# thangvubk/SoftGroup

Measured on AMD Instinct MI355X. Metric: scans/sec ScanNet-v2-like inference (softgroup_scannet.yaml, full forward_test), higher is better.
Workload: dtype f32

## Files before the change

include/softgroup_hip.h:

```cpp
#ifndef SOFTGROUP_HIP_H
#define SOFTGROUP_HIP_H

#include <stddef.h>
#include <stdint.h>

#ifdef __cplusplus
extern "C" {
#endif

typedef void *sg_stream_t;

#define SG_OK 0
#define SG_ERR_ARG (-1)
#define SG_ERR_WORKSPACE (-2)
#define SG_ERR_LAUNCH (-3)
#define SG_ERR_UNSUPPORTED (-4)

#define SG_BALLQUERY_MAX_NEIGHBORS 1000
#define SG_OCTREE_NUM_NODES 585
#define SG_OCTREE_NUM_LEAVES 512
#define SG_LISTS_SORTED 1
#define SG_LISTS_RADIUS 2

int sg_version(void);
// ... 192 lines not shown
  const float *w2;
  const float *w_i;
} sg_unet_block;
typedef struct sg_unet_level {
  int planes, n_blocks;
  const sg_unet_block *blocks;
  const sg_unet_block *tail;
  const float *down_bn_scale, *down_bn_shift, *down_w;
  const float *up_bn_scale, *up_bn_shift, *up_w;
} sg_unet_level;
typedef struct sg_unet_desc {
  int n_levels;
  const sg_unet_level *levels;
  int input_cin;
  const float *input_w;
  const float *out_bn_scale, *out_bn_shift;
  int input_cin_packed;
  int arithmetic;
} sg_unet_desc;
size_t sg_unet_arena_bytes(const sg_unet_desc *desc, int num_rows);
int sg_unet_forward(const sg_unet_desc *desc, const float *feats, const int32_t *indices,
                    int num_rows, const int32_t *spatial_shape_host, float *out, void *arena,
                    size_t arena_bytes, sg_stream_t stream);

typedef struct sg_train_bn {
  const float *weight, *bias;
  float *running_mean, *running_var;
  float momentum, eps;
  float *g_weight, *g_bias;
} sg_train_bn;
typedef struct sg_train_conv {
  const float *w;
  float *g_w;
} sg_train_conv;
typedef struct sg_unet_train_block {
  int cin, cout;
  sg_train_bn bn1, bn2;
  sg_train_conv c1, c2, ci;
} sg_unet_train_block;
typedef struct sg_unet_train_level {
  int planes, n_blocks;
  const sg_unet_train_block *blocks, *tail;
  sg_train_bn down_bn, up_bn;
  sg_train_conv down, up;
} sg_unet_train_level;
typedef struct sg_unet_train_desc {
// ... 418 lines not shown
```

softgroup_amd/_lib.py:

```python
import ctypes as C
import os

_HERE = os.path.dirname(os.path.abspath(__file__))
LIB_PATH = os.path.join(_HERE, 'lib', os.environ.get('SG_LIB_NAME', 'libsoftgroup_hip.so'))

_lib = None

_vp, _i, _f, _i64, _sz, _d = C.c_void_p, C.c_int, C.c_float, C.c_int64, C.c_size_t, C.c_double
_pi32 = C.POINTER(C.c_int32)

SIGNATURES = {
    'sg_version': (_i, []),
    'sg_last_error': (C.c_char_p, []),
    'sg_device_info': (_i, [C.c_char_p, _i, C.POINTER(_i), C.POINTER(_i)]),
    'sg_stream_release': (_i, [_vp]),
    'sg_host_copy_2d': (_i, [_vp, _i64, _vp, _i64, _i64, _i64]),
    'sg_host_cast_f64_f32': (_i, [_vp, _vp, _i64]),
    'sg_host_fill_i64_strided': (_i, [_vp, _i64, _i64, _i64]),
    'sg_host_colmax_i64': (_i, [_vp, _i64, _i64, _vp]),
    'sg_stream_create': (_i, [_vp]),
    'sg_stream_create_priority': (_i, [_vp, _i]),
    'sg_stream_destroy': (_i, [_vp]),
    'sg_voxelize_idx_host': (_i, [_vp, _i, _i, _i, _vp, _pi32, _pi32]),
    'sg_voxelize_idx_fill_host': (_i, [_vp, _i, _i, _i, _vp, _i, _i, _vp, _vp]),
# ... 27 lines not shown
    'sg_get_mask_iou_on_pred': (_i, [_vp, _vp, _vp, _vp, _vp, _i, _i, _vp, _vp]),
    'sg_get_mask_label': (_i, [_vp, _vp, _vp, _vp, _vp, _i, _i, _f, _vp, _vp]),
    'sg_spconv_hash_workspace_bytes': (_sz, [_i]),
    'sg_spconv_subm_rulebook': (_i, [_vp, _i, _pi32, _vp, _vp, _sz, _vp]),
    'sg_spconv_pyramid_workspace_bytes': (_sz, [_i, _i]),
    'sg_spconv_pyramid_rows': (_i, [_vp, _i, _pi32, _i, _vp, _vp, _sz, _vp]),
    'sg_spconv_pyramid_build_workspace_bytes': (_sz, [_vp, _i]),
    'sg_spconv_pyramid_build': (_i, [_vp, _i, _pi32, _i, _vp, _vp, _sz, _vp, _sz, _vp]),
    'sg_spconv_down_build': (_i, [_vp, _i, _pi32, _vp, _vp, _vp, _sz, _vp]),
    'sg_spconv_down_fill': (_i, [_vp, _i, _vp, _i, _vp, _vp, _vp, _sz, _vp]),
    'sg_spconv_inverse_rulebook': (_i, [_vp, _vp, _i, _vp, _vp]),
    'sg_spconv_plan_workspace_bytes': (_sz, [_i]),
    'sg_spconv_plan': (_i, [_vp, _i, _i, _vp, _vp, _vp, _vp, _sz, _vp]),
    'sg_spconv_set_arithmetic': (_i, [_i]),
    'sg_spconv_set_combine': (_i, [_i]),
    'sg_spconv_set_chain': (_i, [_i]),
    'sg_grouping_set_lanes': (_i, [_i]),
    'sg_spconv_chain_stats': (_i, [_vp, _vp]),
    'sg_spconv_profile': (_i, [_i]),
    'sg_spconv_profile_read': (_i, [_vp, _vp]),
    'sg_spconv_profile_detail': (_i, [_vp, _vp, _i, _vp]),
    'sg_unet_arena_bytes': (_sz, [_vp, _i]),
    'sg_unet_forward': (_i, [_vp, _vp, _vp, _i, _vp, _vp, _vp, _sz, _vp]),
    'sg_unet_train_arena_hint': (_sz, [_vp, _i]),
    'sg_unet_train_forward': (_i, [_vp, _vp, _vp, _i, _vp, _vp, _vp, _sz, _vp, _vp, _vp]),
    'sg_unet_train_backward': (_i, [_vp, _vp, _vp, _vp]),
    'sg_unet_train_release': (None, [_vp]),
    'sg_pointwise_heads': (_i, [_vp, _vp, _i, _i, _i, _vp, _vp, _vp, _vp, _vp, _vp, _vp]),
    'sg_spconv_packed_weight_elems': (_sz, [_i, _i, _i]),
    'sg_spconv_pack_weight': (_i, [_vp, _i, _i, _i, _i, _vp, _vp]),
    'sg_spconv_conv_workspace_bytes': (_sz, [_i, _i]),
    'sg_spconv_gather_conv_f32': (_i, [_vp, _i, _vp, _i, _i, _i, _i, _vp, _vp, _vp, _vp, _vp, _vp,
                                       _vp, _vp, _vp, _vp, _vp, _vp, _sz, _vp]),
    'sg_spconv_packed_weight_elems_bf16': (_sz, [_i, _i, _i]),
    'sg_spconv_pack_weight_bf16': (_i, [_vp, _i, _i, _i, _i, _vp, _vp]),
    'sg_spconv_conv_bf16_workspace_bytes': (_sz, [_i, _i]),
    'sg_spconv_gather_conv_bf16': (_i, [_vp, _i, _vp, _i, _i, _i, _i, _vp, _vp, _vp, _vp, _vp, _vp, _sz,
                                        _vp]),
    'sg_spconv_transpose_table': (_i, [_vp, _i, _i, _vp, _vp]),
    'sg_spconv_wgrad_workspace_bytes': (_sz, [_i, _i, _i, _i]),
    'sg_spconv_wgrad': (_i, [_vp, _i, _vp, _i, _vp, _i, _i, _i, _i, _vp, _vp, _sz, _vp]),
    'sg_instance_npoint': (_i, [_vp, _vp, _i64, _i, _i, _f, _i, _vp, _vp]),
    'sg_instance_runs_workspace_bytes': (_sz, [_i, _i]),
    'sg_instance_runs': (_i, [_vp, _vp, _i64, _i, _i, _f, _vp, _i, _i, _i, _vp, _vp, _vp, _i64, _vp, _sz, _vp]),
    'sg_rle_format_bound': (_i64, [_i64, _i]),
    'sg_rle_format_host': (_i, [_vp, _vp, _vp, _i, _vp, _i64, _vp]),
# ... 150 lines not shown
```

softgroup_amd/build.py:

```python
import os
import subprocess
import sys
from concurrent.futures import ThreadPoolExecutor

HERE = os.path.dirname(os.path.abspath(__file__))
CSRC = os.path.join(HERE, 'csrc')
LIBDIR = os.path.join(HERE, 'lib')
OBJDIR = os.path.join(LIBDIR, 'obj')
LIB = os.path.join(LIBDIR, 'libsoftgroup_hip.so')
HIPCC = os.environ.get('HIPCC', '/opt/rocm/bin/hipcc')

SOURCES = [
    ('core.hip', ['-ffp-contract=off']),
    ('seg_ops.hip', ['-ffp-contract=off']),
    ('voxelize_idx.hip', ['-ffp-contract=off']),
    ('ballquery.hip', ['-ffp-contract=off']),
    ('octree.hip', ['-ffp-contract=off']),
    ('bfs.hip', ['-ffp-contract=off']),
    ('spconv_rulebook.hip', ['-ffp-contract=off']),
    ('spconv_conv.hip', ['-mllvm', '-amdgpu-mfma-vgpr-form', '-mllvm', '-amdgpu-atomic-optimizer-strategy=None'] + os.environ.get('SG_CONV_EXTRA_FLAGS', '').split()),
    ('spconv_train.hip', ['-mllvm', '-amdgpu-mfma-vgpr-form']),
    ('unet_exec.hip', ['-ffp-contract=off']),
    ('unet_train.hip', ['-ffp-contract=off']),
    ('instances.hip', ['-ffp-contract=off']),
    ('scan_exec.hip', ['-ffp-contract=off']),
    ('scan_forward.hip', ['-ffp-contract=off']),
    ('heads.hip', ['-ffp-contract=off']),
    ('eval_ops.hip', ['-ffp-contract=off']),
    ('inst_eval.hip', ['-ffp-contract=off']),
    ('det_eval.hip', ['-ffp-contract=off']),
    ('train_data.hip', ['-ffp-contract=off']),
    ('result_io.hip', ['-ffp-contract=off']),
    ('viz_io.hip', ['-ffp-contract=off']),
    ('mask_nms.hip', ['-ffp-contract=off']),
    ('resample.hip', ['-ffp-contract=off']),
    ('losses.hip', ['-ffp-contract=off']),
    ('optim.hip', ['-ffp-contract=off']),
    ('host_ops.cpp', ['-ffp-contract=off']),
]
COMMON = ['-O3', '-std=c++17', '-fPIC', '--offload-arch=gfx950', '-Wall', '-Wno-unused-function',
          '-Wno-unused-result', '-Wno-unused-value']


def _deps_mtime():
    m = 0
# ... 46 lines not shown
```

softgroup_amd/csrc/common.h:

```cpp
#pragma once
#include <hip/hip_runtime.h>
#include <stdint.h>
#include <stdio.h>

#include "../../include/softgroup_hip.h"

namespace sg {

constexpr int kWave = 64;

void set_error(const char *fmt, ...);
int32_t *pinned_words();

inline hipStream_t as_stream(sg_stream_t s) { return reinterpret_cast<hipStream_t>(s); }

inline int check_launch(const char *what) {
  hipError_t e = hipGetLastError();
  if (e != hipSuccess) {
    set_error("%s: %s", what, hipGetErrorString(e));
    return SG_ERR_LAUNCH;
  }
  return SG_OK;
}

// ... 142 lines not shown
  size_t mx = 0;
  for (int i = 0; i < f.n; ++i) mx = f.words[i] > mx ? f.words[i] : mx;
  const int gx = grid_for(static_cast<int64_t>(mx / 4 + 1), 256, 1024);
  fill_many_kernel<<<dim3(gx, f.n), 256, 0, stream>>>(f);
}

extern thread_local int t_conv_arith;
void conv_chain_begin(hipStream_t stream);
bool conv_chain_recording();
int conv_chain_end();
void conv_chain_abort();
int conv_chain_concat(const float *a, const float *b, int64_t rows, int ca, int cb, const float *scale,
                      const float *shift, float *out, float *out_act);
int conv_chain_bn_relu(const float *x, const float *scale, const float *shift, int64_t rows, int c, float *out);
int conv_chain_check_abort(const char *who);
int conv_gather_rows(const void *in, int num_in_rows, const int32_t *nbr, int M_out, int K, int Cin, int Cout,
                     const float *w_k8, const float *post_scale, const float *post_shift, const void *residual,
                     const float *act_scale, const float *act_shift, void *out_act, const int32_t *order,
                     const uint32_t *tile_mask, const int32_t *nbr_tiles, void *out, void *ws, size_t ws_bytes,
                     sg_stream_t stream, int in16, int out16, int res16);
int spconv_wgrad_layout(const void *in, int in_bf16, const void *g_out, int g_bf16, const int32_t *nbr_t, int M_out,
                        int K, int Cin, int Cout, float *dw, int out_oki, void *ws, size_t ws_bytes,
                        sg_stream_t stream);
struct PackJob {
  const float *w;
  float *out;
  int cout, kvol, cin, mode;
};
int spconv_pack_weights(const PackJob *jobs, int n, sg_stream_t stream);
size_t octree_stash_bytes(int n);
int octree_ballquery_count_stash(const float *points, const float *boxes, const int32_t *pt_inds,
                                 const int32_t *pt_start_len, int n, float radius, int32_t *start_len, int32_t *stash,
                                 hipStream_t stream);
int octree_ballquery_fill_stash(const float *points, const float *boxes, const int32_t *pt_inds,
                                const int32_t *pt_start_len, int n, float radius, const int32_t *start_len,
                                const int32_t *stash, int32_t *idx, hipStream_t stream);
void conv_release_stream(int dev, hipStream_t stream);
void unet_release_stream(int dev, hipStream_t stream);
void scan_release_stream(int dev, hipStream_t stream);
void bfs_release_stream(int dev, hipStream_t stream);
constexpr int kBfsGiantMin = 16384;
struct BfsDefer {
  bool deferred = false;
  hipStream_t side = nullptr;
};
void bfs_emit_defer(BfsDefer *d);
// ... 7 lines not shown
```

softgroup_amd/csrc/spconv_conv.hip:

```cpp
#include <stdlib.h>

#include <atomic>
#include <cstdio>
#include <map>
#include <mutex>
#include <utility>
#include <vector>

#include "common.h"

namespace sg {

typedef float f32x16 __attribute__((ext_vector_type(16)));
typedef float f4 __attribute__((ext_vector_type(4)));
typedef float f2 __attribute__((ext_vector_type(2)));
typedef __bf16 bf16x8 __attribute__((ext_vector_type(8)));
typedef __bf16 bf16x2 __attribute__((ext_vector_type(2)));

__device__ __forceinline__ void split3(const float (&x)[8], bf16x8 &h, bf16x8 &m, bf16x8 &l) {
#pragma unroll
  for (int j = 0; j < 4; ++j) {
    const f2 v = {x[2 * j], x[2 * j + 1]};
    const bf16x2 hh = __builtin_convertvector(v, bf16x2);
    const f2 r = v - __builtin_convertvector(hh, f2);
    const bf16x2 mm = __builtin_convertvector(r, bf16x2);
    const f2 r2 = r - __builtin_convertvector(mm, f2);
    const bf16x2 ll = __builtin_convertvector(r2, bf16x2);
    h[2 * j] = hh[0]; h[2 * j + 1] = hh[1];
    m[2 * j] = mm[0]; m[2 * j + 1] = mm[1];
    l[2 * j] = ll[0]; l[2 * j + 1] = ll[1];
  }
}
__device__ __forceinline__ bf16x8 round_bf16(const float (&x)[8]) {
  bf16x8 h;
#pragma unroll
  for (int j = 0; j < 4; ++j) {
    const f2 v = {x[2 * j], x[2 * j + 1]};
    const bf16x2 hh = __builtin_convertvector(v, bf16x2);
    h[2 * j] = hh[0]; h[2 * j + 1] = hh[1];
  }
  return h;
}
__device__ __forceinline__ uint16_t bf16_rne(float x) {
  const uint32_t u = __builtin_bit_cast(uint32_t, x);
  return static_cast<uint16_t>((u + 0x7fffu + ((u >> 16) & 1u)) >> 16);
}
__device__ __forceinline__ float bf16_f32(uint16_t b) {
  return __builtin_bit_cast(float, static_cast<uint32_t>(b) << 16);
}

#ifndef SG_WHATIF
#define SG_WHATIF 0
#endif

constexpr int kTileRows = 32;
// ... 1402 lines not shown
#define SG_B16_DEPTH 2
#endif
#ifndef SG_B16_WPE_PLUS
#define SG_B16_WPE_PLUS 0
#endif
template <int CK, int WPE, int NBW, int WV, int AT>
constexpr PersistentFn r16_variant() {
  if constexpr (AT) return gather_conv_persistent_kernel<CK, SG_B16_DEPTH, 0, WPE + SG_B16_WPE_PLUS, NBW, 2, WV, 1, 1>;
  else return nullptr;
}
#define SG_SPLIT_VARIANT(CK, DEPTH, WPE, NBW, WV, AT)                                            \
  {gather_conv_persistent_kernel<CK, DEPTH, 0, WPE, NBW, 1, WV, AT>,                              \
   gather_conv_persistent_kernel<CK, DEPTH, 1, WPE, NBW, 1, WV, AT>,                              \
   gather_conv_persistent_kernel<CK, SG_B16_DEPTH, 0, WPE + SG_B16_WPE_PLUS, NBW, 2, WV, AT>,     \
   r16_variant<CK, WPE, NBW, WV, AT>(), NBW, WV, CK, AT, 0, 0, 0, 0}
constexpr int kSplitVariants = 9;
static SplitVariant g_split_variants[kSplitVariants] = {
    SG_SPLIT_VARIANT(32, 2, 2, 2, 2, 1),  SG_SPLIT_VARIANT(32, 2, 3, 1, 2, 1),
    SG_SPLIT_VARIANT(32, 2, 2, 2, 4, 1),  SG_SPLIT_VARIANT(32, 2, 3, 1, 4, 1), SG_SPLIT_VARIANT(32, 2, 1, 1, 8, 1),
    SG_SPLIT_VARIANT(16, 2, 3, 2, 4, 0),  SG_SPLIT_VARIANT(16, 2, 4, 1, 4, 0), SG_SPLIT_VARIANT(16, 2, 2, 1, 8, 0),
    SG_SPLIT_VARIANT(16, 2, 1, 1, 16, 0),
};

static int launch_persistent_split(ConvArgs a, int num_tiles, long long in_bytes, long long w_bytes,
                                   hipStream_t stream, bool b16, bool in16) {
  static int num_cu = 0;
  static std::once_flag once;
  std::call_once(once, [] {
    int dev = 0;
    hipGetDevice(&dev);
    hipDeviceGetAttribute(&num_cu, hipDeviceAttributeMultiprocessorCount, dev);
    if (num_cu <= 0) num_cu = 256;
    auto prepare = [](SplitVariant &v) {
      v.lds = static_cast<size_t>(v.wv) * v.nbw * 16 * 64 * sizeof(float) + 2 * kMetaInts * sizeof(int32_t) + 16 +
              (v.at ? static_cast<size_t>(v.wv) * 4096 : 0);
      int o = 0;
      hipOccupancyMaxActiveBlocksPerMultiprocessor(&o, v.fn, 64 * v.wv, v.lds);
      v.occ = o < 1 ? 1 : o;
      o = 0;
      hipOccupancyMaxActiveBlocksPerMultiprocessor(&o, v.fn_b16, 64 * v.wv, v.lds);
      v.occ_b16 = o < 1 ? 1 : o;
      o = 0;
      if (v.fn_r16) hipOccupancyMaxActiveBlocksPerMultiprocessor(&o, v.fn_r16, 64 * v.wv, v.lds);
      v.occ_r16 = o < 1 ? 1 : o;
    };
    for (SplitVariant &v : g_split_variants) prepare(v);
  });
  static const int nbw_env = getenv("SG_CONV_NBW") ? atoi(getenv("SG_CONV_NBW")) : 2;
  static const int wv_env = getenv("SG_CONV_WV") ? atoi(getenv("SG_CONV_WV")) : 0;
  static const float min_rounds = getenv("SG_CONV_ROUNDS") ? atof(getenv("SG_CONV_ROUNDS")) : 2.5f;
  static const int at_env = getenv("SG_CONV_AT") ? atoi(getenv("SG_CONV_AT")) : 1;
  const int NB = (a.Cout + 31) / 32;
  const unsigned long long row_bytes = (in16 ? 2ull : 4ull) * a.Cin;
  const unsigned absent_at = static_cast<unsigned>((0xFFFFFFull * row_bytes) & 0xFFFFFFFFull);
  const int use_at = ((at_env != 0 || in16) && a.Cin % 32 == 0 && in_bytes / static_cast<long long>(row_bytes) < (1LL << 24) - 1 &&
                      static_cast<long long>(absent_at) >= in_bytes) ? 1 : 0;
  if (in16 && (!use_at || !b16)) {
    set_error("sg_unet_forward(bf16 rows): a layer with %d input channels / %lld input bytes cannot take the line-wise bf16 gather",
              a.Cin, in_bytes);
    return SG_ERR_ARG;
  }
  int pick = -1;
  static const int w2_max = getenv("SG_CONV_W2_MAX") ? atoi(getenv("SG_CONV_W2_MAX")) : 108;
  static const int w2_nbw = getenv("SG_CONV_W2_NBW") ? atoi(getenv("SG_CONV_W2_NBW")) : 2;
  static const float w2_rounds = getenv("SG_CONV_W2_ROUNDS") ? atof(getenv("SG_CONV_W2_ROUNDS")) : 1.5f;
  const bool use_w2 = wv_env == 2 || (wv_env == 0 && a.K * (a.Cin / 32) <= w2_max);
  for (int i = 0; i < kSplitVariants; ++i) {
    const SplitVariant &v = g_split_variants[i];
    if (v.at != use_at) continue;
    if (v.wv == 2 && (!use_w2 || a.ksplit > 1 || v.nbw > w2_nbw)) continue;
    if (a.ksplit > 1) {
      if (v.nbw == 1 && v.wv == 4) { pick = i; break; }
      continue;
    }
    pick = i;
    if (v.nbw == 2 && (a.Cout % 64 != 0 || nbw_env < 2)) continue;
    if (wv_env && v.wv != wv_env) continue;
    const long long units = static_cast<long long>(num_tiles) * (NB / v.nbw);
    if (wv_env || units >= static_cast<long long>((v.wv == 2 ? w2_rounds : min_rounds) * num_cu * (in16 ? v.occ_r16 : b16 ? v.occ_b16 : v.occ))) {
      pick = i;
      break;
    }
  }
  const bool chain_layer = t_chain.mode != 0 && use_at != 0;
  if (chain_layer) {
    for (int i = 0; i < kSplitVariants; ++i)
      if (g_split_variants[i].at == 1 && g_split_variants[i].nbw == 1 && g_split_variants[i].wv == kChainWV) pick = i;
  }
  const SplitVariant &v = g_split_variants[pick];
  a.col_units = NB / v.nbw;
  a.blocks_per_unit = v.nbw;
  const long long units = static_cast<long long>(num_tiles) * a.col_units * a.ksplit;
  a.num_units = static_cast<int>(units);
  auto magic = [](unsigned d) { return d <= 1 ? 0u : static_cast<unsigned>((1ULL << 32) / d) + 1u; };
  a.magic_upt = magic(static_cast<unsigned>(a.col_units * a.ksplit));
  a.magic_cu = magic(static_cast<unsigned>(a.col_units));
  a.magic_nsl = magic(static_cast<unsigned>(in16 ? (a.Cin + 63) / 64 : a.Cin / v.ck));
  if (t_chain.mode == 2) {
    if (chain_layer && !in16 && !a.out16 && !a.res16 && (a.ksplit == 1 || a.done != nullptr) && stream == t_chain.stream) {
      ChainStep st = {};
      st.kind = 0;
      st.in = a.in; st.w = a.w; st.post_scale = a.post_scale; st.post_shift = a.post_shift; st.residual = a.residual;
      st.act_scale = a.act_scale; st.act_shift = a.act_shift; st.out_act = a.out_act; st.order = a.order;
      st.tile_mask = a.tile_mask; st.nbr_tiles = a.nbr_tiles; st.out = a.out; st.done = a.done; st.out_final = a.out_final;
      st.M_out = a.M_out; st.K = a.K; st.Cin = a.Cin; st.Cout = a.Cout; st.col_units = a.col_units;
      st.ksplit = a.ksplit; st.k_per_split = a.k_per_split; st.num_units = a.num_units;
      st.magic_upt = a.magic_upt; st.magic_cu = a.magic_cu; st.magic_nsl = a.magic_nsl;
      st.in_bytes = static_cast<unsigned>(in_bytes); st.w_bytes = static_cast<unsigned>(w_bytes);
      return chain_push(st, b16, a.K > 1);
    }
    const int rc = chain_flush();
    if (rc != SG_OK) return rc;
// ... 16 lines not shown
  }
  static const char *trace_env = getenv("SG_CONV_TRACE");
  if (trace_env) {
    const size_t nb = static_cast<size_t>(units) * kWavesPerWg * 8 * sizeof(unsigned long long);
    unsigned long long *dbuf = nullptr;
    hipMalloc(&dbuf, nb);
    hipMemsetAsync(dbuf, 0, nb, stream);
    a.trace = dbuf;
    v.fn_trace<<<static_cast<int>(g), 64 * v.wv, v.lds, stream>>>(a, ib, wb);
    hipStreamSynchronize(stream);
    std::vector<unsigned long long> h(nb / 8);
    hipMemcpy(h.data(), dbuf, nb, hipMemcpyDeviceToHost);
    hipFree(dbuf);
    if (FILE *f = fopen(trace_env, "ab")) {
      long long hdr[8] = {a.M_out, a.K, a.Cin, a.Cout, units, a.col_units, v.wv, g};
      fwrite(hdr, 8, 8, f);
      fwrite(h.data(), 8, h.size(), f);
      fclose(f);
    }
  } else {
    v.fn<<<static_cast<int>(g), 64 * v.wv, v.lds, stream>>>(a, ib, wb);
  }
  return check_launch("sg_spconv_gather_conv_f32(split)");
}


}

using namespace sg;

extern "C" {

int sg_spconv_set_arithmetic(int mode) {
  SG_REQUIRE(mode >= -1 && mode <= 2, "sg_spconv_set_arithmetic: mode must be -1, 0, 1 or 2");
  g_arith_override = mode;
  return SG_OK;
}

int sg_spconv_set_combine(int mode) {
  SG_REQUIRE(mode >= -1 && mode <= 1, "sg_spconv_set_combine: mode must be -1, 0 or 1");
  g_combine_override = mode;
  return SG_OK;
}

int sg_spconv_set_chain(int mode) {
  SG_REQUIRE(mode >= -1 && mode <= 1, "sg_spconv_set_chain: mode must be -1, 0 or 1");
// ... 276 lines not shown
```

softgroup_amd/csrc/unet_exec.hip:

```cpp
#include <map>
#include <mutex>
#include <utility>
#include <vector>

#include <stdlib.h>

#include "common.h"
#include "radix_sort.h"
#include "unet_common.h"

namespace sg {

__global__ void __launch_bounds__(256) batch_max_kernel(const int32_t *__restrict__ indices, int M,
                                                       int32_t *__restrict__ bmax) {
  int m = 0;
  for (int i = blockIdx.x * 256 + threadIdx.x; i < M; i += gridDim.x * 256) m = max(m, indices[4 * i]);
#pragma unroll
  for (int o = 32; o > 0; o >>= 1) m = max(m, __shfl_xor(m, o, 64));
  if ((threadIdx.x & 63) == 0 && m > 0) atomicMax(bmax, m);
}
__device__ __forceinline__ uint64_t spread3(uint32_t v) {
  uint64_t x = v & 0x1fffffu;
  x = (x | (x << 32)) & 0x1f00000000ffffull;
  x = (x | (x << 16)) & 0x1f0000ff0000ffull;
// ... 332 lines not shown

  int conv(const float *in, int in_rows, const Plan &p, int cin, int cout, const float *w,
           const float *post_s, const float *post_b, const float *residual, const Act &act, float *out,
           bool in_f32 = false, bool out_f32 = false) {
    if (p.rows == 0) return SG_OK;
    const size_t m = ar.mark();
    const size_t nb = sg_spconv_conv_workspace_bytes(p.rows, cout);
    void *ws = nullptr;
    if (nb > 256) {
      ws = ar.take<char>(nb);
    }
    const int rc = !r16 ? sg_spconv_gather_conv_f32(in, in_rows, p.nbr, p.rows, p.kvol, cin, cout, w, post_s,
                                                    post_b, residual, act.scale, act.shift, act.out, p.order,
                                                    p.tile_mask, p.nbr_tiles, out, ws, ws ? nb : 0, stream)
                        : conv_gather_rows(in, in_rows, p.nbr, p.rows, p.kvol, cin, cout, w, post_s, post_b, residual,
                                           act.scale, act.shift, act.out, p.order, p.tile_mask, p.nbr_tiles, out, ws,
                                           ws ? nb : 0, stream, in_f32 ? 0 : 1, out_f32 ? 0 : 1, 1);
    ar.release(m);
    return rc;
  }

  int block(const sg_unet_block &b, const float *x, const float *xa, int rows, const Plan &subm,
            const Plan &ident, const float *post_s, const float *post_b, const Act &next, float *out,
            bool out_f32 = false) {
    const size_t m = ar.mark();
    const float *shortcut = x;
    if (b.w_i != nullptr) {
      SG_ALLOC(sc, float, fsz(static_cast<size_t>(rows) * b.cout));
      SG_TRY(conv(x, rows, ident, b.cin, b.cout, b.w_i, nullptr, nullptr, nullptr, Act(), sc));
      shortcut = sc;
    }
    SG_ALLOC(h, float, fsz(static_cast<size_t>(rows) * b.cout));
    SG_TRY(conv(xa, rows, subm, b.cin, b.cout, b.w1, b.bn2_scale, b.bn2_shift, nullptr, Act(), h));
    SG_TRY(conv(h, rows, subm, b.cout, b.cout, b.w2, post_s, post_b, shortcut, next, out, false, out_f32));
    ar.release(m);
    return SG_OK;
  }

  int level(int l, const float *x, const float *xa, const float *pre_in, int pre_cin,
            const float *post_s, const float *post_b, float *out) {
    const sg_unet_level &L = d->levels[l];
    const int c = L.planes;
    const bool deeper = l + 1 < d->n_levels;
    const size_t m0 = ar.mark();
    const LevelIdx &I = idx[l];
    const int rows = I.rows;
    const Plan &subm = I.subm, &ident = I.ident;
    const size_t feat = fsz(static_cast<size_t>(rows ? rows : 1) * c);
    if (pre_in != nullptr) {
      SG_ALLOC(x0, float, feat);
// ... 32 lines not shown
      }
      const bool fin = last && !deeper;
      SG_TRY(block(L.blocks[i], cur, cur_a, rows, subm, ident, fin ? post_s : nullptr,
                   fin ? post_b : nullptr, next, dst, fin && l == 0));
      cur = dst;
      cur_a = next.out;
    }
    if (deeper) {
      const int c2 = d->levels[l + 1].planes;
      const int rows2 = idx[l + 1].rows;
      const Plan &down = I.down, &up = I.up;
      const sg_unet_level &L2 = d->levels[l + 1];
      const size_t feat2 = fsz(static_cast<size_t>(rows2 ? rows2 : 1) * c2);
      SG_ALLOC(y, float, feat2);
      SG_ALLOC(ya, float, feat2);
      const Act ay{L2.blocks[0].bn1_scale, L2.blocks[0].bn1_shift, ya};
      SG_ALLOC(z, float, feat2);
      {
        ChainScope chain(*this, chain_from(l + 1));
        SG_TRY(conv(cur_a, rows, down, c, c2, L.down_w, nullptr, nullptr, nullptr, ay, y));
        SG_TRY(level(l + 1, y, ya, nullptr, 0, L.up_bn_scale, L.up_bn_shift, z));
        SG_TRY(chain.close());
      }
      SG_ALLOC(cat, float, 2 * feat);
      SG_ALLOC(cata, float, 2 * feat);
      {
        const size_t m = ar.mark();
        SG_ALLOC(upf, float, feat);
        SG_TRY(conv(z, rows2, up, c2, c, L.up_w, nullptr, nullptr, nullptr, Act(), upf));
        if (rows && r16)
          concat2_bf16_kernel<<<grid_for(static_cast<int64_t>(rows) * (2 * c / 4), 256), 256, 0, as_stream(stream)>>>(
              reinterpret_cast<const uint2 *>(cur), reinterpret_cast<const uint2 *>(upf), rows, c / 4, c / 4,
              reinterpret_cast<const float4 *>(L.tail[0].bn1_scale), reinterpret_cast<const float4 *>(L.tail[0].bn1_shift),
              reinterpret_cast<uint2 *>(cat), reinterpret_cast<uint2 *>(cata));
        else if (rows && conv_chain_recording())
          SG_TRY(conv_chain_concat(cur, upf, rows, c, c, L.tail[0].bn1_scale, L.tail[0].bn1_shift, cat, cata));
        else if (rows)
          concat2_kernel<<<grid_for(static_cast<int64_t>(rows) * (2 * c / 4), 256), 256, 0, as_stream(stream)>>>(
              reinterpret_cast<const float4 *>(cur), reinterpret_cast<const float4 *>(upf), rows, c / 4,
              c / 4, reinterpret_cast<const float4 *>(L.tail[0].bn1_scale),
              reinterpret_cast<const float4 *>(L.tail[0].bn1_shift), reinterpret_cast<float4 *>(cat),
              reinterpret_cast<float4 *>(cata));
        ar.release(m);
      }
      cur = cat;
      cur_a = cata;
      for (int i = 0; i < L.n_blocks; ++i) {
        const bool last = i == L.n_blocks - 1;
        float *dst = out;
        Act next;
        if (!last) {
          SG_ALLOC(t, float, feat);
          SG_ALLOC(ta, float, feat);
          dst = t;
          next = Act{L.tail[i + 1].bn1_scale, L.tail[i + 1].bn1_shift, ta};
        }
        SG_TRY(block(L.tail[i], cur, cur_a, rows, subm, ident, last ? post_s : nullptr,
                     last ? post_b : nullptr, next, dst, last && l == 0));
        cur = dst;
        cur_a = next.out;
      }
    }
    ar.release(m0);
    return check_launch("sg_unet_forward");
  }
};

static size_t level_index_bytes(size_t rows, size_t rows_next, bool deeper) {
  const size_t t = (rows + 31) / 32, t2 = (rows_next + 31) / 32;
  size_t b = align_up(rows * 4 * 4) + align_up(rows * 27 * 4) +
             align_up(t * 32 * 4) + align_up((t + SG_PLAN_HIST_WORDS) * 4) + align_up(t * 32 * 27 * 4);
  if (deeper)
    b += align_up(rows * 4) + align_up(rows_next * 8 * 4) + align_up(rows * 8 * 4) +
         align_up(t2 * 32 * 4) + align_up((t2 + SG_PLAN_HIST_WORDS) * 4) + align_up(t2 * 32 * 8 * 4) +
         align_up(t * 32 * 4) + align_up((t + SG_PLAN_HIST_WORDS) * 4) + align_up(t * 32 * 8 * 4);
  return b + 4096;
}
size_t unet_index_bytes(int L, int num_rows) {
  const size_t rows = static_cast<size_t>(num_rows > 0 ? num_rows : 1);
  size_t total = (1 << 20) + sg_spconv_pyramid_workspace_bytes(num_rows, L) +
                 (L + 1) * (align_up(rows * 4) + align_up(rows / 8 + 256) + 4096);
// ... 129 lines not shown
```

Baseline: 424.7.

## Fuse decoder up-conv, concat, BN-ReLU and shortcut conv into one kernel

Adds a single kernel for each decoder level's entry. It computes the inverse (up) sparse conv with split-bf16 MFMA, writes the BN+ReLU activated concatenation, and computes the 1x1 shortcut conv over the concatenated features without materialising the raw concat buffer. The goal is to cut the separate up-conv launch, the concat kernel and the identity-conv launch, along with their intermediate global memory round trips. It is gated on row count (default above 6144), the f32 split arithmetic, and no chain recording or bf16 rows, so it only runs on large levels. The shortcut is now computed from the up-conv tile held in LDS, which adds code complexity and possibly a different accumulation order.

```diff
diff --git a/include/softgroup_hip.h b/include/softgroup_hip.h
--- a/include/softgroup_hip.h
+++ b/include/softgroup_hip.h
@@ -238,6 +238,13 @@
 int sg_unet_forward(const sg_unet_desc *desc, const float *feats, const int32_t *indices,
                     int num_rows, const int32_t *spatial_shape_host, float *out, void *arena,
                     size_t arena_bytes, sg_stream_t stream);
+
+int sg_unet_decoder_entry(const float *z, int rows2, const float *cur, int rows, const int32_t *up_order,
+                          const uint32_t *up_tile_mask, const int32_t *up_nbr_tiles, int c2, int c,
+                          const float *up_w, const float *w_i, const float *bn_scale, const float *bn_shift,
+                          float *cata, float *sc, sg_stream_t stream);
+int sg_unet_set_fused_entry(int mode, int min_rows);
+int64_t sg_unet_fused_entry_launches(void);
 
 typedef struct sg_train_bn {
   const float *weight, *bias;
diff --git a/softgroup_amd/_lib.py b/softgroup_amd/_lib.py
--- a/softgroup_amd/_lib.py
+++ b/softgroup_amd/_lib.py
@@ -73,6 +73,9 @@
     'sg_spconv_profile_detail': (_i, [_vp, _vp, _i, _vp]),
     'sg_unet_arena_bytes': (_sz, [_vp, _i]),
     'sg_unet_forward': (_i, [_vp, _vp, _vp, _i, _vp, _vp, _vp, _sz, _vp]),
+    'sg_unet_decoder_entry': (_i, [_vp, _i, _vp, _i, _vp, _vp, _vp, _i, _i, _vp, _vp, _vp, _vp, _vp, _vp, _vp]),
+    'sg_unet_set_fused_entry': (_i, [_i, _i]),
+    'sg_unet_fused_entry_launches': (_i64, []),
     'sg_unet_train_arena_hint': (_sz, [_vp, _i]),
     'sg_unet_train_forward': (_i, [_vp, _vp, _vp, _i, _vp, _vp, _vp, _sz, _vp, _vp, _vp]),
     'sg_unet_train_backward': (_i, [_vp, _vp, _vp, _vp]),
diff --git a/softgroup_amd/build.py b/softgroup_amd/build.py
--- a/softgroup_amd/build.py
+++ b/softgroup_amd/build.py
@@ -21,6 +21,7 @@
     ('spconv_conv.hip', ['-mllvm', '-amdgpu-mfma-vgpr-form', '-mllvm', '-amdgpu-atomic-optimizer-strategy=None'] + os.environ.get('SG_CONV_EXTRA_FLAGS', '').split()),
     ('spconv_train.hip', ['-mllvm', '-amdgpu-mfma-vgpr-form']),
     ('unet_exec.hip', ['-ffp-contract=off']),
+    ('unet_entry.hip', ['-ffp-contract=off', '-mllvm', '-amdgpu-mfma-vgpr-form']),
     ('unet_train.hip', ['-ffp-contract=off']),
     ('instances.hip', ['-ffp-contract=off']),
     ('scan_exec.hip', ['-ffp-contract=off']),
diff --git a/softgroup_amd/csrc/common.h b/softgroup_amd/csrc/common.h
--- a/softgroup_amd/csrc/common.h
+++ b/softgroup_amd/csrc/common.h
@@ -188,6 +188,11 @@
 int spconv_wgrad_layout(const void *in, int in_bf16, const void *g_out, int g_bf16, const int32_t *nbr_t, int M_out,
                         int K, int Cin, int Cout, float *dw, int out_oki, void *ws, size_t ws_bytes,
                         sg_stream_t stream);
+bool conv_split_shape(int num_in_rows, int M_out, int K, int Cin, int Cout, int *wv, bool *one_unit);
+bool conv_profile_begin(hipStream_t stream, int M_out, int K, int Cin, int Cout, int num_in_rows);
+void conv_profile_end(hipStream_t stream);
+bool unet_entry_usable(int rows2, int rows, int c2, int c);
+bool unet_entry_wanted(int rows);
 struct PackJob {
   const float *w;
   float *out;
diff --git a/softgroup_amd/csrc/mfma_split.h b/softgroup_amd/csrc/mfma_split.h
--- /dev/null
+++ b/softgroup_amd/csrc/mfma_split.h
@@ -0,0 +1,27 @@
+#pragma once
+#include "common.h"
+
+namespace sg {
+
+typedef float f32x16 __attribute__((ext_vector_type(16)));
+typedef float f4 __attribute__((ext_vector_type(4)));
+typedef float f2 __attribute__((ext_vector_type(2)));
+typedef __bf16 bf16x8 __attribute__((ext_vector_type(8)));
+typedef __bf16 bf16x2 __attribute__((ext_vector_type(2)));
+
+__device__ __forceinline__ void split3(const float (&x)[8], bf16x8 &h, bf16x8 &m, bf16x8 &l) {
+#pragma unroll
+  for (int j = 0; j < 4; ++j) {
+    const f2 v = {x[2 * j], x[2 * j + 1]};
+    const bf16x2 hh = __builtin_convertvector(v, bf16x2);
+    const f2 r = v - __builtin_convertvector(hh, f2);
+    const bf16x2 mm = __builtin_convertvector(r, bf16x2);
+    const f2 r2 = r - __builtin_convertvector(mm, f2);
+    const bf16x2 ll = __builtin_convertvector(r2, bf16x2);
+    h[2 * j] = hh[0]; h[2 * j + 1] = hh[1];
+    m[2 * j] = mm[0]; m[2 * j + 1] = mm[1];
+    l[2 * j] = ll[0]; l[2 * j + 1] = ll[1];
+  }
+}
+
+}
diff --git a/softgroup_amd/csrc/spconv_conv.hip b/softgroup_amd/csrc/spconv_conv.hip
--- a/softgroup_amd/csrc/spconv_conv.hip
+++ b/softgroup_amd/csrc/spconv_conv.hip
@@ -8,29 +8,10 @@
 #include <vector>
 
 #include "common.h"
+#include "mfma_split.h"
 
 namespace sg {
 
-typedef float f32x16 __attribute__((ext_vector_type(16)));
-typedef float f4 __attribute__((ext_vector_type(4)));
-typedef float f2 __attribute__((ext_vector_type(2)));
-typedef __bf16 bf16x8 __attribute__((ext_vector_type(8)));
-typedef __bf16 bf16x2 __attribute__((ext_vector_type(2)));
-
-__device__ __forceinline__ void split3(const float (&x)[8], bf16x8 &h, bf16x8 &m, bf16x8 &l) {
-#pragma unroll
-  for (int j = 0; j < 4; ++j) {
-    const f2 v = {x[2 * j], x[2 * j + 1]};
-    const bf16x2 hh = __builtin_convertvector(v, bf16x2);
-    const f2 r = v - __builtin_convertvector(hh, f2);
-    const bf16x2 mm = __builtin_convertvector(r, bf16x2);
-    const f2 r2 = r - __builtin_convertvector(mm, f2);
-    const bf16x2 ll = __builtin_convertvector(r2, bf16x2);
-    h[2 * j] = hh[0]; h[2 * j + 1] = hh[1];
-    m[2 * j] = mm[0]; m[2 * j + 1] = mm[1];
-    l[2 * j] = ll[0]; l[2 * j + 1] = ll[1];
-  }
-}
 __device__ __forceinline__ bf16x8 round_bf16(const float (&x)[8]) {
   bf16x8 h;
 #pragma unroll
@@ -1479,11 +1460,12 @@
     SG_SPLIT_VARIANT(16, 2, 1, 1, 16, 0),
 };
 
-static int launch_persistent_split(ConvArgs a, int num_tiles, long long in_bytes, long long w_bytes,
-                                   hipStream_t stream, bool b16, bool in16) {
-  static int num_cu = 0;
+struct SplitPick { int variant, use_at; };
+static int g_split_num_cu = 0;
+static SplitPick pick_split_variant(const ConvArgs &a, int num_tiles, long long in_bytes, bool b16, bool in16) {
+  int &num_cu = g_split_num_cu;
   static std::once_flag once;
-  std::call_once(once, [] {
+  std::call_once(once, [&num_cu] {
     int dev = 0;
     hipGetDevice(&dev);
     hipDeviceGetAttribute(&num_cu, hipDeviceAttributeMultiprocessorCount, dev);
@@ -1512,11 +1494,7 @@
   const unsigned absent_at = static_cast<unsigned>((0xFFFFFFull * row_bytes) & 0xFFFFFFFFull);
   const int use_at = ((at_env != 0 || in16) && a.Cin % 32 == 0 && in_bytes / static_cast<long long>(row_bytes) < (1LL << 24) - 1 &&
                       static_cast<long long>(absent_at) >= in_bytes) ? 1 : 0;
-  if (in16 && (!use_at || !b16)) {
-    set_error("sg_unet_forward(bf16 rows): a layer with %d input channels / %lld input bytes cannot take the line-wise bf16 gather",
-              a.Cin, in_bytes);
-    return SG_ERR_ARG;
-  }
+  if (in16 && (!use_at || !b16)) return SplitPick{-1, use_at};
   int pick = -1;
   static const int w2_max = getenv("SG_CONV_W2_MAX") ? atoi(getenv("SG_CONV_W2_MAX")) : 108;
   static const int w2_nbw = getenv("SG_CONV_W2_NBW") ? atoi(getenv("SG_CONV_W2_NBW")) : 2;
@@ -1544,7 +1522,21 @@
     for (int i = 0; i < kSplitVariants; ++i)
       if (g_split_variants[i].at == 1 && g_split_variants[i].nbw == 1 && g_split_variants[i].wv == kChainWV) pick = i;
   }
-  const SplitVariant &v = g_split_variants[pick];
+  return SplitPick{pick, use_at};
+}
+
+static int launch_persistent_split(ConvArgs a, int num_tiles, long long in_bytes, long long w_bytes,
+                                   hipStream_t stream, bool b16, bool in16) {
+  const SplitPick sp = pick_split_variant(a, num_tiles, in_bytes, b16, in16);
+  if (sp.variant < 0) {
+    set_error("sg_unet_forward(bf16 rows): a layer with %d input channels / %lld input bytes cannot take the line-wise bf16 gather",
+              a.Cin, in_bytes);
+    return SG_ERR_ARG;
+  }
+  const int num_cu = g_split_num_cu;
+  const bool chain_layer = t_chain.mode != 0 && sp.use_at != 0;
+  const SplitVariant &v = g_split_variants[sp.variant];
+  const int NB = (a.Cout + 31) / 32;
   a.col_units = NB / v.nbw;
   a.blocks_per_unit = v.nbw;
   const long long units = static_cast<long long>(num_tiles) * a.col_units * a.ksplit;
@@ -1607,6 +1599,44 @@
     v.fn<<<static_cast<int>(g), 64 * v.wv, v.lds, stream>>>(a, ib, wb);
   }
   return check_launch("sg_spconv_gather_conv_f32(split)");
+}
+
+bool conv_profile_begin(hipStream_t stream, int M_out, int K, int Cin, int Cout, int num_in_rows) {
+  if (!g_conv_prof.enabled) return false;
+  hipEventRecord(g_conv_prof.take(), stream);
+  for (int v : {M_out, K, Cin, Cout, num_in_rows}) g_conv_prof.dims.push_back(v);
+  return true;
+}
+void conv_profile_end(hipStream_t stream) { hipEventRecord(g_conv_prof.take(), stream); }
+
+bool conv_split_shape(int num_in_rows, int M_out, int K, int Cin, int Cout, int *wv, bool *one_unit) {
+  static const int split_env = getenv("SG_CONV_SPLIT") ? atoi(getenv("SG_CONV_SPLIT")) : 1;
+  static const int split_min_cin = getenv("SG_CONV_SPLIT_MIN_CIN") ? atoi(getenv("SG_CONV_SPLIT_MIN_CIN")) : 16;
+  static const int target_env = getenv("SG_CONV_TARGET") ? atoi(getenv("SG_CONV_TARGET")) : 0;
+  const int arith_ov = t_conv_arith >= 0 ? t_conv_arith : g_arith_override.load(std::memory_order_relaxed);
+  if ((arith_ov >= 0 ? arith_ov : split_env) != 1 || Cin < split_min_cin || Cin % 32 != 0 || Cout % 32 != 0) return false;
+  if (M_out <= 0 || num_in_rows <= 0 || K < 1 || K > kMaxK) return false;
+  const long long in_bytes = static_cast<long long>(num_in_rows) * Cin * 4;
+  const int num_tiles = (M_out + kTileRows - 1) / kTileRows;
+  if (in_bytes >= (1LL << 31) || static_cast<long long>(M_out) * Cout * 4 * kMaxK >= (1LL << 32) ||
+      static_cast<long long>(num_tiles) * kTileRows * K * 4 >= (1LL << 31))
+    return false;
+  const int target = target_env > 0 ? target_env : 1024;
+  const long long waves = static_cast<long long>(num_tiles) * (Cout / 32) * kWavesPerWg;
+  int ksplit = 1;
+  if (waves < target / 2 && sg_spconv_conv_workspace_bytes(M_out, Cout) > 256) {
+    const long long want = (target / 2 + waves - 1) / waves;
+    ksplit = static_cast<int>(want < K ? want : K);
+    const int k_per_split = (K + ksplit - 1) / ksplit;
+    ksplit = (K + k_per_split - 1) / k_per_split;
+  }
+  ConvArgs a = {};
+  a.M_out = M_out; a.K = K; a.Cin = Cin; a.Cout = Cout; a.ksplit = ksplit;
+  const SplitPick sp = pick_split_variant(a, num_tiles, in_bytes, false, false);
+  if (sp.variant < 0 || !sp.use_at) return false;
+  *wv = g_split_variants[sp.variant].wv;
+  *one_unit = ksplit == 1;
+  return true;
 }
 
 
diff --git a/softgroup_amd/csrc/unet_entry.hip b/softgroup_amd/csrc/unet_entry.hip
--- /dev/null
+++ b/softgroup_amd/csrc/unet_entry.hip
@@ -0,0 +1,298 @@
+#include <stdlib.h>
+
+#include <atomic>
+
+#include "common.h"
+#include "mfma_split.h"
+
+namespace sg {
+
+namespace {
+
+constexpr unsigned kPast = 0x80000000u;
+
+struct EntryArgs {
+  const float *z, *cur, *up_w, *w_i, *bn_scale, *bn_shift;
+  const int32_t *order;
+  const uint32_t *tile_mask;
+  const int32_t *nbr_tiles;
+  float *cata, *sc;
+  int c2, num_tiles, up_wv, id_wv;
+  unsigned z_bytes, cur_bytes, upw_bytes, wi_bytes;
+};
+
+constexpr int kWaveLds = 4096 + 1024 + 128;
+
+template <int NB>
+__global__ void __launch_bounds__(64 * NB) decoder_entry_kernel(EntryArgs p) {
+  constexpr int C = 32 * NB;
+  __shared__ __attribute__((aligned(16))) char smem[NB * (4096 + kWaveLds)];
+  const int wave = NB == 1 ? 0 : __builtin_amdgcn_readfirstlane(threadIdx.x >> 6), lane = threadIdx.x & 63;
+  const int tile = blockIdx.x;
+  const int arow = lane & 31, ahalf = lane >> 5;
+  f4 *ub = reinterpret_cast<f4 *>(smem);
+  char *mine = smem + NB * 4096 + wave * kWaveLds;
+  f4 *tr = reinterpret_cast<f4 *>(mine);
+  int32_t *nb_l = reinterpret_cast<int32_t *>(mine + 4096);
+  int32_t *row_l = nb_l + 256;
+
+  reinterpret_cast<int4 *>(nb_l)[lane] = reinterpret_cast<const int4 *>(p.nbr_tiles + static_cast<size_t>(tile) * 256)[lane];
+  if (lane < 32) row_l[lane] = p.order[static_cast<size_t>(tile) * 32 + lane];
+  const uint32_t mask = __builtin_amdgcn_readfirstlane(p.tile_mask[tile]) & 0xffu;
+
+  const __amdgpu_buffer_rsrc_t rs_z = __builtin_amdgcn_make_buffer_rsrc(const_cast<float *>(p.z), 0, p.z_bytes, 0x00020000);
+  const __amdgpu_buffer_rsrc_t rs_cur = __builtin_amdgcn_make_buffer_rsrc(const_cast<float *>(p.cur), 0, p.cur_bytes, 0x00020000);
+  const __amdgpu_buffer_rsrc_t rs_wu = __builtin_amdgcn_make_buffer_rsrc(const_cast<float *>(p.up_w), 0, p.upw_bytes, 0x00020000);
+  const __amdgpu_buffer_rsrc_t rs_wi = __builtin_amdgcn_make_buffer_rsrc(const_cast<float *>(p.w_i), 0, p.wi_bytes, 0x00020000);
+
+  const int lrow = lane >> 3, chunk = lane & 7;
+  int rq[4];
+#pragma unroll
+  for (int q = 0; q < 4; ++q) rq[q] = row_l[8 * q + lrow];
+  unsigned cur_off[4];
+#pragma unroll
+  for (int q = 0; q < 4; ++q)
+    cur_off[q] = rq[q] >= 0 ? static_cast<unsigned>(rq[q]) * static_cast<unsigned>(C * 4) + chunk * 16u : kPast;
+
+  struct Slice { f4 a[4]; f4 b[6]; };
+  const int v_w = (ahalf * C + wave * 32 + arow) * 16;
+  auto load_w = [&](const __amdgpu_buffer_rsrc_t &rs, int s_w, int plane_bytes, Slice &S) {
+#pragma unroll
+    for (int sl = 0; sl < 2; ++sl)
+#pragma unroll
+      for (int pl = 0; pl < 3; ++pl)
+        S.b[sl * 3 + pl] = __builtin_bit_cast(f4, __builtin_amdgcn_raw_buffer_load_b128(
+                                                      rs, v_w, s_w + sl * (2 * C * 16) + pl * plane_bytes, 0));
+  };
+  auto mma = [&](const f4 *blk, const Slice &S, f32x16 &acc) {
+    f4 fr[2][2];
+#pragma unroll
+    for (int sl = 0; sl < 2; ++sl)
+#pragma unroll
+      for (int j = 0; j < 2; ++j) fr[sl][j] = blk[arow * 8 + ((sl * 4 + ahalf * 2 + j) ^ ((arow >> 1) & 7))];
+#pragma unroll
+    for (int sl = 0; sl < 2; ++sl) {
+      const float af[8] = {fr[sl][0][0], fr[sl][0][1], fr[sl][0][2], fr[sl][0][3],
+                           fr[sl][1][0], fr[sl][1][1], fr[sl][1][2], fr[sl][1][3]};
+      bf16x8 ah, am, al;
+      split3(af, ah, am, al);
+      const bf16x8 bh = __builtin_bit_cast(bf16x8, S.b[sl * 3 + 0]);
+      const bf16x8 bm = __builtin_bit_cast(bf16x8, S.b[sl * 3 + 1]);
+      const bf16x8 bl = __builtin_bit_cast(bf16x8, S.b[sl * 3 + 2]);
+      acc = __builtin_amdgcn_mfma_f32_32x32x16_bf16(al, bh, acc, 0, 0, 0);
+      acc = __builtin_amdgcn_mfma_f32_32x32x16_bf16(am, bm, acc, 0, 0, 0);
+      acc = __builtin_amdgcn_mfma_f32_32x32x16_bf16(ah, bl, acc, 0, 0, 0);
+      acc = __builtin_amdgcn_mfma_f32_32x32x16_bf16(am, bh, acc, 0, 0, 0);
+      acc = __builtin_amdgcn_mfma_f32_32x32x16_bf16(ah, bm, acc, 0, 0, 0);
+      acc = __builtin_amdgcn_mfma_f32_32x32x16_bf16(ah, bh, acc, 0, 0, 0);
+    }
+  };
+  auto to_lines = [&](const Slice &S) {
+#pragma unroll
+    for (int q = 0; q < 4; ++q) {
+      const int r = 8 * q + lrow;
+      tr[r * 8 + (chunk ^ ((r >> 1) & 7))] = S.a[q];
+    }
+  };
+  f32x16 tot, acc;
+  auto zero = [](f32x16 &v) {
+#pragma unroll
+    for (int r = 0; r < 16; ++r) v[r] = 0.f;
+  };
+  auto run = [&](int n, int per, auto &&load, auto &&compute) {
+    zero(tot);
+    zero(acc);
+    Slice S0, S1;
+    if (n > 0) load(0, S0);
+    int gend = per, w = 0;
+    auto join = [&](int it) {
+      if (it + 1 != gend && it + 1 != n) return;
+      if (w == 0) tot = acc;
+      else tot += acc;
+      zero(acc);
+      ++w;
+      gend += per;
+    };
+    for (int it = 0; it < n; it += 2) {
+      if (it + 1 < n) load(it + 1, S1);
+      compute(it, S0);
+      join(it);
+      if (it + 1 < n) {
+        if (it + 2 < n) load(it + 2, S0);
+        compute(it + 1, S1);
+        join(it + 1);
+      }
+    }
+  };
+
+  {
+    const int ns = p.c2 >> 5, c8 = p.c2 >> 3;
+    const int plane_bytes = 8 * c8 * C * 16, planes_at = 2 * plane_bytes;
+    const unsigned pitch = static_cast<unsigned>(p.c2) * 4u;
+    const int items = __builtin_popcount(mask) * ns;
+    const int per = (items + p.up_wv - 1) / p.up_wv;
+    int nk = -1, ks = ns;
+    uint32_t mm = mask;
+    run(items, per,
+        [&](int, Slice &S) {
+          if (++ks >= ns) {
+            ks = 0;
+            nk = __builtin_ctz(mm);
+            mm &= mm - 1u;
+          }
+#pragma unroll
+          for (int q = 0; q < 4; ++q) {
+            const int src = nb_l[(8 * q + lrow) * 8 + nk];
+            const unsigned off = src >= 0 ? static_cast<unsigned>(src) * pitch + chunk * 16u : kPast;
+            S.a[q] = __builtin_bit_cast(f4, __builtin_amdgcn_raw_buffer_load_b128(rs_z, off, ks * 128, 0));
+          }
+          load_w(rs_wu, planes_at + (nk * c8 + ks * 4) * C * 16, plane_bytes, S);
+        },
+        [&](int, const Slice &S) {
+          to_lines(S);
+          mma(tr, S, acc);
+        });
+  }
+
+  {
+    constexpr int ITEMS = 2 * NB, c8 = 2 * C / 8;
+    constexpr int plane_bytes = c8 * C * 16, planes_at = 2 * plane_bytes;
+    const f4 *scale4 = reinterpret_cast<const f4 *>(p.bn_scale), *shift4 = reinterpret_cast<const f4 *>(p.bn_shift);
+    const f4 sc_a = scale4[wave * 8 + chunk], sh_a = shift4[wave * 8 + chunk];
+    const f4 sc_b = scale4[(NB + wave) * 8 + chunk], sh_b = shift4[(NB + wave) * 8 + chunk];
+    auto store_act = [&](const f4 (&a)[4], const f4 &s4, const f4 &h4, int it) {
+#pragma unroll
+      for (int q = 0; q < 4; ++q) {
+        if (rq[q] < 0) continue;
+        f4 v;
+#pragma unroll
+        for (int j = 0; j < 4; ++j) v[j] = fmaxf(fmaf(a[q][j], s4[j], h4[j]), 0.f);
+        *reinterpret_cast<f4 *>(p.cata + static_cast<size_t>(rq[q]) * (2 * C) + it * 32 + chunk * 4) = v;
+      }
+    };
+    {
+      float *blk = reinterpret_cast<float *>(ub + wave * 256);
+#pragma unroll
+      for (int reg = 0; reg < 16; ++reg) {
+        const int r = (reg & 3) + 8 * (reg >> 2) + 4 * ahalf;
+        blk[r * 32 + (((arow >> 2) ^ ((r >> 1) & 7)) << 2) + (arow & 3)] = tot[reg] + 0.f;
+      }
+    }
+    if (NB > 1) __syncthreads();
+    {
+      f4 a[4];
+#pragma unroll
+      for (int q = 0; q < 4; ++q) {
+        const int r = 8 * q + lrow;
+        a[q] = ub[wave * 256 + r * 8 + (chunk ^ ((r >> 1) & 7))];
+      }
+      store_act(a, sc_b, sh_b, NB + wave);
+    }
+    const int per = (ITEMS + p.id_wv - 1) / p.id_wv;
+    run(ITEMS, per,
+        [&](int it, Slice &S) {
+          if (it < NB) {
+#pragma unroll
+            for (int q = 0; q < 4; ++q)
+              S.a[q] = __builtin_bit_cast(f4, __builtin_amdgcn_raw_buffer_load_b128(rs_cur, cur_off[q], it * 128, 0));
+          }
+          load_w(rs_wi, planes_at + it * 4 * C * 16, plane_bytes, S);
+        },
+        [&](int it, const Slice &S) {
+          if (it < NB) {
+            if (it == wave) store_act(S.a, sc_a, sh_a, it);
+            to_lines(S);
+            mma(tr, S, acc);
+          } else {
+            mma(ub + (it - NB) * 256, S, acc);
+          }
+        });
+#pragma unroll
+    for (int reg = 0; reg < 16; ++reg) {
+      const int row = row_l[(reg & 3) + 8 * (reg >> 2) + 4 * ahalf];
+      if (row >= 0) p.sc[static_cast<size_t>(row) * C + wave * 32 + arow] = tot[reg] + 0.f;
+    }
+  }
+}
+
+std::atomic<int> g_fused_mode{-1}, g_fused_rows{-1};
+std::atomic<long long> g_entry_launches{0};
+
+}
+
+bool unet_entry_usable(int rows2, int rows, int c2, int c) {
+  if (rows <= 0 || rows2 < 0 || c % 32 != 0 || c < 32 || c > 128 || c2 % 32 != 0 || c2 < 32) return false;
+  if (static_cast<long long>(rows) * 2 * c * 4 >= (1LL << 31) || static_cast<long long>(rows2) * c2 * 4 >= (1LL << 31)) return false;
+  int wv = 0;
+  bool one = false;
+  return conv_split_shape(rows, rows, 1, 2 * c, c, &wv, &one) &&
+         (rows2 == 0 || conv_split_shape(rows2, rows, 8, c2, c, &wv, &one));
+}
+
+bool unet_entry_wanted(int rows) {
+  static const int mode_env = getenv("SG_UNET_FUSED_ENTRY") ? atoi(getenv("SG_UNET_FUSED_ENTRY")) : 1;
+  static const int rows_env = getenv("SG_UNET_FUSED_ENTRY_ROWS") ? atoi(getenv("SG_UNET_FUSED_ENTRY_ROWS")) : 6144;
+  const int mode = g_fused_mode.load(std::memory_order_relaxed), lim = g_fused_rows.load(std::memory_order_relaxed);
+  return (mode >= 0 ? mode : mode_env) != 0 && rows > (lim >= 0 ? lim : rows_env);
+}
+
+}
+
+using namespace sg;
+
+extern "C" {
+
+int sg_unet_set_fused_entry(int mode, int min_rows) {
+  SG_REQUIRE(mode >= -1 && mode <= 1, "sg_unet_set_fused_entry: mode must be -1, 0 or 1");
+  g_fused_mode = mode;
+  g_fused_rows = min_rows < 0 ? -1 : min_rows;
+  return SG_OK;
+}
+
+int sg_unet_decoder_entry(const float *z, int rows2, const float *cur, int rows, const int32_t *up_order,
+                          const uint32_t *up_tile_mask, const int32_t *up_nbr_tiles, int c2, int c,
+                          const float *up_w, const float *w_i, const float *bn_scale, const float *bn_shift,
+                          float *cata, float *sc, sg_stream_t stream) {
+  SG_REQUIRE(rows >= 0 && rows2 >= 0, "sg_unet_decoder_entry: bad row counts");
+  if (rows == 0) return SG_OK;
+  SG_REQUIRE(cur && up_order && up_tile_mask && up_nbr_tiles && up_w && w_i && bn_scale && bn_shift && cata && sc &&
+                 (z || rows2 == 0),
+             "sg_unet_decoder_entry: null argument");
+  SG_REQUIRE(reinterpret_cast<uintptr_t>(up_nbr_tiles) % 16 == 0 && reinterpret_cast<uintptr_t>(cur) % 16 == 0 &&
+                 reinterpret_cast<uintptr_t>(z) % 16 == 0 && reinterpret_cast<uintptr_t>(cata) % 16 == 0 &&
+                 reinterpret_cast<uintptr_t>(bn_scale) % 16 == 0 && reinterpret_cast<uintptr_t>(bn_shift) % 16 == 0 &&
+                 reinterpret_cast<uintptr_t>(up_w) % 16 == 0 && reinterpret_cast<uintptr_t>(w_i) % 16 == 0,
+             "sg_unet_decoder_entry: buffers must be 16-byte aligned");
+  SG_REQUIRE(unet_entry_usable(rows2, rows, c2, c),
+             "sg_unet_decoder_entry: needs c %% 32 == 0, 32 <= c <= 128, c2 %% 32 == 0, buffers below 2 GB and the "
+             "split-precision conv arithmetic (rows=%d rows2=%d c=%d c2=%d)", rows, rows2, c, c2);
+  EntryArgs a;
+  a.z = z; a.cur = cur; a.up_w = up_w; a.w_i = w_i; a.bn_scale = bn_scale; a.bn_shift = bn_shift;
+  a.order = up_order; a.tile_mask = up_tile_mask; a.nbr_tiles = up_nbr_tiles; a.cata = cata; a.sc = sc;
+  a.c2 = c2;
+  a.num_tiles = (rows + 31) / 32;
+  bool one = false;
+  a.up_wv = 2;
+  a.id_wv = 2;
+  conv_split_shape(rows, rows, 1, 2 * c, c, &a.id_wv, &one);
+  if (rows2 > 0) conv_split_shape(rows2, rows, 8, c2, c, &a.up_wv, &one);
+  a.z_bytes = static_cast<unsigned>(static_cast<size_t>(rows2) * c2 * 4);
+  a.cur_bytes = static_cast<unsigned>(static_cast<size_t>(rows) * c * 4);
+  a.upw_bytes = static_cast<unsigned>(sg_spconv_packed_weight_elems(8, c2, c) * 4);
+  a.wi_bytes = static_cast<unsigned>(sg_spconv_packed_weight_elems(1, 2 * c, c) * 4);
+  hipStream_t st = as_stream(stream);
+  const bool timed = conv_profile_begin(st, rows, 8, c2, c, rows2);
+  switch (c / 32) {
+    case 1: decoder_entry_kernel<1><<<a.num_tiles, 64, 0, st>>>(a); break;
+    case 2: decoder_entry_kernel<2><<<a.num_tiles, 128, 0, st>>>(a); break;
+    case 3: decoder_entry_kernel<3><<<a.num_tiles, 192, 0, st>>>(a); break;
+    default: decoder_entry_kernel<4><<<a.num_tiles, 256, 0, st>>>(a); break;
+  }
+  if (timed) conv_profile_end(st);
+  g_entry_launches.fetch_add(1, std::memory_order_relaxed);
+  return check_launch("sg_unet_decoder_entry");
+}
+
+int64_t sg_unet_fused_entry_launches(void) { return g_entry_launches.load(std::memory_order_relaxed); }
+
+}
diff --git a/softgroup_amd/csrc/unet_exec.hip b/softgroup_amd/csrc/unet_exec.hip
--- a/softgroup_amd/csrc/unet_exec.hip
+++ b/softgroup_amd/csrc/unet_exec.hip
@@ -378,10 +378,12 @@
 
   int block(const sg_unet_block &b, const float *x, const float *xa, int rows, const Plan &subm,
             const Plan &ident, const float *post_s, const float *post_b, const Act &next, float *out,
-            bool out_f32 = false) {
+            bool out_f32 = false, const float *ready_sc = nullptr) {
     const size_t m = ar.mark();
     const float *shortcut = x;
-    if (b.w_i != nullptr) {
+    if (ready_sc != nullptr) {
+      shortcut = ready_sc;
+    } else if (b.w_i != nullptr) {
       SG_ALLOC(sc, float, fsz(static_cast<size_t>(rows) * b.cout));
       SG_TRY(conv(x, rows, ident, b.cin, b.cout, b.w_i, nullptr, nullptr, nullptr, Act(), sc));
       shortcut = sc;
@@ -460,9 +462,24 @@
         SG_TRY(level(l + 1, y, ya, nullptr, 0, L.up_bn_scale, L.up_bn_shift, z));
         SG_TRY(chain.close());
       }
-      SG_ALLOC(cat, float, 2 * feat);
+      const sg_unet_block &t0 = L.tail[0];
+      const bool fused = rows > 0 && unet_entry_wanted(rows) && !r16 && !conv_chain_recording() && t0.w_i != nullptr &&
+                         t0.cin == 2 * c && t0.cout == c && unet_entry_usable(rows2, rows, c2, c);
+      float *cat = nullptr, *sc0 = nullptr;
+      if (fused) {
+        sc0 = ar.take<float>(feat);
+      } else {
+        cat = ar.take<float>(2 * feat);
+      }
+      if (cat == nullptr && sc0 == nullptr) {
+        set_error("sg_unet_forward: arena too small (%zu bytes, need more than %zu)", ar.cap, ar.off);
+        return SG_ERR_WORKSPACE;
+      }
       SG_ALLOC(cata, float, 2 * feat);
-      {
+      if (fused) {
+        SG_TRY(sg_unet_decoder_entry(z, rows2, cur, rows, up.order, up.tile_mask, up.nbr_tiles, c2, c, L.up_w, t0.w_i,
+                                     t0.bn1_scale, t0.bn1_shift, cata, sc0, stream));
+      } else {
         const size_t m = ar.mark();
         SG_ALLOC(upf, float, feat);
         SG_TRY(conv(z, rows2, up, c2, c, L.up_w, nullptr, nullptr, nullptr, Act(), upf));
@@ -494,7 +511,7 @@
           next = Act{L.tail[i + 1].bn1_scale, L.tail[i + 1].bn1_shift, ta};
         }
         SG_TRY(block(L.tail[i], cur, cur_a, rows, subm, ident, last ? post_s : nullptr,
-                     last ? post_b : nullptr, next, dst, last && l == 0));
+                     last ? post_b : nullptr, next, dst, last && l == 0, i == 0 ? sc0 : nullptr));
         cur = dst;
         cur_a = next.out;
       }
```

After: 436.6 (median of 6 runs). 2.8% higher.
